# mitsuba-renderer/mitsuba

Measured on AMD Instinct MI355X. Metric: Msamples/s, higher is better.
Workload: dtype f32; 1 GPU; cornell_1024x1024_256spp; scene=cornell_box, triangles=32, width=1024, height=1024, spp=256, integrator=path_hip maxDepth=-1 rrDepth=5, rfilter=gaussian stddev 0.5, sampler=ctr seed 0, block_size=32, parallelism=1 GPU

## Files before the change

### mitsuba_amd/csrc/k_mega.h

```cpp

#ifndef MEGA_PROFILE
#define MEGA_PROFILE 0
#endif
#ifndef MEGA_MB_DIAG
#define MEGA_MB_DIAG 0
#endif
#ifndef MEGA_MB_CLASSES
#define MEGA_MB_CLASSES 1
#endif
#ifndef MEGA_MB_THRESH
#define MEGA_MB_THRESH 40
#endif
#ifndef MEGA_MB_PATIENCE
#define MEGA_MB_PATIENCE 6
#endif
#define MB_NR 48u
template <bool RBOX, uint32_t N> struct MailboxEntry {
    enum { SEQ_ROW = 64 };
    enum { HEAD = 0, DIR = 4, THR = RBOX ? 8 : 7, MIS = THR + 4, ID = MIS + 2, PIXEL, K, STATE, ACCUM, LAST = ACCUM + 3, SEQ = 22 };
    static_assert(LAST < SEQ && SEQ + 2 == MB_DW && MB_DW == 24, "a mailbox entry: the path's state lies below the two rows of the sequence index, which end the MB_DW rows k_pool.h sizes the boxes with");
    static __device__ __forceinline__ void put(uint32_t *x, int row, float f) { x[row * N] = pm_to_bits(f); }
    static __device__ __forceinline__ float get(const uint32_t *x, int row) { return pm_from_bits(x[row * N]); }
    static __device__ __forceinline__ void put4(uint32_t *x, int row, const float4 &f) { put(x, row, f.x); put(x, row + 1, f.y); put(x, row + 2, f.z); put(x, row + 3, f.w); }
    static __device__ __forceinline__ float4 get4(const uint32_t *x, int row) { return make_float4(get(x, row), get(x, row + 1), get(x, row + 2), get(x, row + 3)); }
    template <bool QMC> static __device__ __forceinline__ void store(uint32_t *x, const PathVertex &v, const float4 &accum, const uint32_t *seq) {
        if (RBOX) { put4(x, HEAD, v.rayO); put4(x, DIR, v.rayD); }
        else { put4(x, HEAD, v.hit); put(x, DIR, v.rayD.x); put(x, DIR + 1, v.rayD.y); put(x, DIR + 2, v.rayD.z); }
        put4(x, THR, v.thr);
        put(x, MIS, v.mis.x); put(x, MIS + 1, v.mis.y);
        x[ID * N] = v.id; x[PIXEL * N] = v.pixel; x[K * N] = v.k; x[STATE * N] = v.state;
        put4(x, ACCUM, accum);
        if (QMC) { x[SEQ * N] = seq[0]; x[(SEQ + 1) * N] = seq[SEQ_ROW]; }
    }
    template <bool QMC> static __device__ __forceinline__ void load(const uint32_t *x, PathVertex &v, float4 &accum, uint32_t *seq) {
        if (RBOX) { v.rayO = get4(x, HEAD); v.rayD = get4(x, DIR); }
        else { v.hit = get4(x, HEAD); v.rayD = make_float4(get(x, DIR), get(x, DIR + 1), get(x, DIR + 2), 0.0f); }
        v.thr = get4(x, THR);
        v.mis = make_float2(get(x, MIS), get(x, MIS + 1));
        v.id = x[ID * N]; v.pixel = x[PIXEL * N]; v.k = x[K * N]; v.state = x[STATE * N];
        accum = get4(x, ACCUM);
        if (QMC) { seq[0] = x[SEQ * N]; seq[SEQ_ROW] = x[(SEQ + 1) * N]; }
    }
};
typedef MailboxEntry<false, MB_NS> SBoxEntry;
typedef MailboxEntry<true, MB_NR> RBoxEntry;
static_assert((BLOCK / 64u) * BAL_WAVE_BYTES + MB_DW * MB_NS * sizeof(uint32_t) <= MEGA_DEAL_DWORDS * BLOCK * sizeof(uint32_t), "the S-box lies behind the work lists in the region phip.hip sizes with MEGA_DEAL_DWORDS");
#define MEGA_CHUNK_MAX 4096u
#define MEGA_CHUNK_MIN 64u

enum { MC_SAMPLES = 0, MC_VERTICES, MC_RAYS, MC_NODE, MC_TRI, MC_SH_RAYS, MC_SH_NODE, MC_SH_TRI, MC_COUNT };

template <int MM, bool STRICT, int FLAT ,
          bool QMC ,
          bool DIRECT = false > __global__ __launch_bounds__(BLOCK, MEGA_WAVES) void k_mega(DevScene S, MegaParams M, RenderConst rc, float4 *L) {
    constexpr bool WIDE = FLAT >= 4;
    constexpr bool MAILBOX = MM != 0 && !WIDE && !DIRECT;
    __shared__ uint32_t mbR[MAILBOX ? MB_DW * MB_NR : 1u];
    __shared__ uint32_t mbState[MAILBOX ? MB_NS + MB_NR : 1u];
    __shared__ int mbLive;
    constexpr bool WCNT = (WIDE || (MAILBOX && QMC)) && !MEGA_PROFILE && !MEGA_MB_DIAG;
    __shared__ uint32_t ldsCount[WCNT ? 1 : MC_COUNT][WCNT ? 1 : BLOCK];
#define MEGA_COUNT(row, amount) ldsCount[row][threadIdx.x] += (uint32_t) (amount)
    enum { WC_SAMPLES = 0, WC_VERTICES, WC_RAYS, WC_STEPS, WC_SH_RAYS, WC_SH_STEPS, WC_COUNT };
    __shared__ unsigned long long wcnt[WCNT || WIDE ? BLOCK / 64 : 1][WC_COUNT];
    constexpr int RQ_ROWS = QMC ? 10 : 8;
    __shared__ uint32_t ldsRegen[BLOCK / 64][RQ_ROWS][64];
    __shared__ uint32_t ldsSeq[QMC ? BLOCK / 64 : 1][2][64];
    constexpr uint32_t WAVE_BYTES = WP_WAVE_BYTES;
    unsigned char *wideDeal = g_smem + widePoolDealOffset(M.nodeCache);
    float4 *ldsTriShade = (float4 *) (g_smem + recordsLdsEndOf(S));
    float *ldsEm = WIDE ? (float *) (wideDeal + (BLOCK / 64u) * WAVE_BYTES + (MAILBOX ? MB_DW * MB_NS * sizeof(uint32_t) : 0u))
                        : (float *) (ldsTriShade + (size_t) S.nTriangles * TRISHADE_FLOAT4S);
    DevMaterial *ldsMat = (DevMaterial *) (ldsEm + ((S.emitterTabSize + 3u) & ~3u));
    ShadeTables tab = stageShadeTables<FLAT != 5>(S, ldsEm, ldsMat);
    tab.T.t = ldsEm; tab.materials = FLAT == 5 ? S.materials : ldsMat;
    float4 *ldsFlat = (float4 *) (((uintptr_t) (ldsMat + S.nMaterials) + 15u) & ~(uintptr_t) 15u);
    if (!WIDE) for (uint32_t i = threadIdx.x; i < 2u * S.nFlatLeaves; i += BLOCK) ldsFlat[i] = S.flatLeaves[i];
    lds_cf4 *flat = (lds_cf4 *) ldsFlat; (void) flat;
    if (!WIDE) {
        for (uint32_t i = threadIdx.x; i < S.nTriangles * TRISHADE_FLOAT4S; i += BLOCK) ldsTriShade[i] = S.triShade[i];
        S.triShade = ldsTriShade;
    }
    if (MAILBOX) { if (threadIdx.x < MB_NS + MB_NR) mbState[threadIdx.x] = 0u; if (threadIdx.x == 0u) mbLive = 0; }
    lds_cf4 *const ldsTris = (lds_cf4 *) (g_smem + (size_t) S.dealDwords * BLOCK * sizeof(uint32_t)); (void) ldsTris;
    WidePool wpool;
    if (WIDE) setupWidePool(S, M.nodeCache, g_smem, M.spill + (size_t) blockIdx.x * BLOCK * SPILL_DEPTH, (uint32_t) __builtin_amdgcn_readfirstlane((int) (threadIdx.x >> 6)), wpool);
    else stageRecords(S, g_smem);

    const uint32_t waveId = blockIdx.x * (BLOCK / 64) + (uint32_t) __builtin_amdgcn_readfirstlane((int) (threadIdx.x >> 6)), lane = __lane_id();
    unsigned long long next = 0, end = 0;
    const uint32_t waveInBlock = (uint32_t) __builtin_amdgcn_readfirstlane((int) (threadIdx.x >> 6));
    unsigned char *const waveDeal = wideDeal + waveInBlock * WAVE_BYTES;
    WaveBalance wb = waveBalanceAt(g_smem, waveInBlock);
    if (WIDE) { wb.slot = (lds_u64 *) waveDeal; wb.list = (lds_u16 *) (waveDeal + 2u * 64u * 8u); }
    bool poolOverflow = false;
    uint32_t qHead = 0, qCount = 0;
    V3 camO;
    { V3 d_; float mn_, mx_; cameraRay(S.cam, 0.5f, 0.5f, camO, d_, mn_, mx_); }
    bool exhausted = rc.totalIds == 0;
    uint32_t *mbS = WIDE ? (uint32_t *) (wideDeal + (BLOCK / 64u) * WAVE_BYTES)
                         : (uint32_t *) (g_smem + (BLOCK / 64u) * BAL_WAVE_BYTES);
    const bool server = MAILBOX && waveInBlock == 0u;
    bool haveHit = false;
    uint32_t idleSpins = 0, patience = 0, idleSig = 0;
    bool mbTimedOut = false;
#if MEGA_MB_DIAG
    uint32_t dgDeposit = 0, dgLocal = 0, dgWithdrawn = 0, dgKept = 0, dgServerPass = 0, dgClientPass = 0, dgRefill = 0, dgServerRegen = 0;
#endif
    auto mbAssign = [&](bool wants, bool avail, uint32_t &e) -> bool {
        const unsigned long long am = __ballot(avail), wm = __ballot(wants);
        lds_u32 *map = (lds_u32 *) wb.slot;
        if (avail) map[__builtin_amdgcn_mbcnt_hi((uint32_t) (am >> 32), __builtin_amdgcn_mbcnt_lo((uint32_t) am, 0u))] = lane;
        BAL_SYNC();
        const uint32_t rw = __builtin_amdgcn_mbcnt_hi((uint32_t) (wm >> 32), __builtin_amdgcn_mbcnt_lo((uint32_t) wm, 0u));
        const bool got = wants && rw < (uint32_t) __popcll(am);
        e = got ? map[rw] : 0u;
        BAL_SYNC();
        return got;
    };

    bool alive = false;
    PathVertex v; v.id = v.pixel = v.k = v.state = 0;
    v.hit = v.rayO = v.rayD = v.thr = make_float4(0, 0, 0, 0); v.mis = make_float2(0, 0);
    float4 accum = make_float4(0, 0, 0, 0);
    float4 camHit = make_float4(0, 0, 0, 0);
    if (!WCNT) {
#pragma unroll
        for (int i = 0; i < MC_COUNT; ++i) ldsCount[WCNT ? 0 : i][WCNT ? 0 : threadIdx.x] = 0;
    }
    unsigned long long *const wc = wcnt[(WCNT || WIDE) ? waveInBlock : 0u];
    if ((WCNT || WIDE) && lane < (uint32_t) WC_COUNT) wc[lane] = 0ull;
    auto wcAdd = [&](int row, uint32_t perLane, bool shiftHigh) {
        uint32_t t = perLane;
        t += (uint32_t) __builtin_amdgcn_update_dpp(0, (int) t, 0x111, 0xf, 0xf, true);
        t += (uint32_t) __builtin_amdgcn_update_dpp(0, (int) t, 0x112, 0xf, 0xf, true);
        t += (uint32_t) __builtin_amdgcn_update_dpp(0, (int) t, 0x114, 0xf, 0xf, true);
        t += (uint32_t) __builtin_amdgcn_update_dpp(0, (int) t, 0x118, 0xf, 0xf, true);
        t += (uint32_t) __builtin_amdgcn_update_dpp(0, (int) t, 0x142, 0xa, 0xf, false);
        t += (uint32_t) __builtin_amdgcn_update_dpp(0, (int) t, 0x143, 0xc, 0xf, false);
        if (lane == 63u) wc[row] += shiftHigh ? ((unsigned long long) t << 32) : (unsigned long long) t;
    };
    bool cPush = false, cPend = false;
    float4 cPark = make_float4(0, 0, 0, 0);
    ShadowEntry cSh; cSh.e0 = cSh.e1 = cSh.e2 = make_float4(0, 0, 0, 0);

#if MEGA_PROFILE
    unsigned long long pfT[4] = { 0, 0, 0, 0 }, pfL[4] = { 0, 0, 0, 0 }, pfIter = 0;
// ... 64 lines not shown
                        const bool stop = __hip_atomic_load(M.cancel, __ATOMIC_RELAXED, __HIP_MEMORY_SCOPE_SYSTEM) != 0;
                        if (seen < rc.totalIds && !stop) {
                            const unsigned long long share = (rc.totalIds - seen) / (2ull * M.nWaves);
                            chunk = (uint32_t) (share > MEGA_CHUNK_MAX ? MEGA_CHUNK_MAX : (share < MEGA_CHUNK_MIN ? MEGA_CHUNK_MIN : share));
                            chunk &= ~63u;
                            if (MAILBOX) {
                                atomicAdd(&mbLive, (int) chunk);
                                __builtin_amdgcn_fence(__ATOMIC_SEQ_CST, "workgroup");
                            }
                            base = atomicAdd(M.nextId, (unsigned long long) chunk);
                        } else {
                            base = rc.totalIds;
                        }
                    }
                    const uint32_t blo = __builtin_amdgcn_readfirstlane((uint32_t) base), bhi = __builtin_amdgcn_readfirstlane((uint32_t) (base >> 32));
                    chunk = __builtin_amdgcn_readfirstlane(chunk);
                    next = ((unsigned long long) bhi << 32) | blo;
                    end = next + chunk; if (end > rc.totalIds) end = rc.totalIds;
                    if (MAILBOX && lane == 0u && chunk) {
                        const unsigned long long granted = end > next ? end - next : 0ull;
                        if (granted < chunk) atomicSub(&mbLive, (int) (chunk - granted));
                    }
                    if (next >= end) { exhausted = true; break; }
                }
                const unsigned long long id = next + lane;
                uint32_t px = 0, py = 0, k = 0;
                const bool valid = id < end && decodeId(rc, S.film, id, px, py, k);
                const unsigned long long vmask = __ballot(valid);
                if (MAILBOX) { const int skipped = __popcll(__ballot(id < end && !valid)); if (skipped && lane == 0u) atomicSub(&mbLive, skipped); }
                if (valid) {
                    const uint32_t pos = __builtin_amdgcn_mbcnt_hi((uint32_t) (vmask >> 32), __builtin_amdgcn_mbcnt_lo((uint32_t) vmask, 0u));
                    const uint32_t pixel = py * (uint32_t) S.film.width + px;
                    const V2 jit = streamJitter<QMC>(rc, pixel, k, (uint32_t) S.film.width);
                    if (QMC && rc.jitter) rc.jitter[id] = make_float2(jit.x, jit.y);
                    const float sx = (float) px + jit.x, sy = (float) py + jit.y;
                    V3 o, d; float mint, maxt;
                    cameraRay(S.cam, sx, sy, o, d, mint, maxt);
                    uint32_t *q = &ldsRegen[waveInBlock][0][pos];
                    q[0 * 64] = pm_to_bits(mint);
                    q[1 * 64] = pm_to_bits(d.x); q[2 * 64] = pm_to_bits(d.y); q[3 * 64] = pm_to_bits(d.z); q[4 * 64] = pm_to_bits(maxt);
                    q[5 * 64] = (uint32_t) id; q[6 * 64] = pixel; q[7 * 64] = k;
                    if (QMC) {
                        const uint64_t sidx = isSequenceSampler(rc.sampler) ? seqIndex(rc, k, px, py) : 0ull;
                        q[8 * 64] = (uint32_t) sidx; q[9 * 64] = (uint32_t) (sidx >> 32);
                    }
                }
                qHead = 0u; qCount = (uint32_t) __popcll(vmask);
                next = (end - next < 64ull) ? end : next + 64ull;
                if (qCount == 0u) continue;
            }
            const uint32_t rank = __builtin_amdgcn_mbcnt_hi((uint32_t) (want >> 32), __builtin_amdgcn_mbcnt_lo((uint32_t) want, 0u));
            if (!alive && rank < qCount) {
                const uint32_t *q = &ldsRegen[waveInBlock][0][qHead + rank];
                v.rayO = make_float4(camO.x, camO.y, camO.z, pm_from_bits(q[0 * 64]));
                v.rayD = make_float4(pm_from_bits(q[1 * 64]), pm_from_bits(q[2 * 64]), pm_from_bits(q[3 * 64]), pm_from_bits(q[4 * 64]));
                v.id = q[5 * 64]; v.pixel = q[6 * 64]; v.k = q[7 * 64];
                if (QMC) { ldsSeq[waveInBlock][0][lane] = q[8 * 64]; ldsSeq[waveInBlock][1][lane] = q[9 * 64]; }
                v.thr = make_float4(1.0f, 1.0f, 1.0f, 1.0f);
                v.mis = make_float2(0.0f, 0.0f);
                v.state = 1u | F_ALIVE | F_EMITTED | F_FIRST;
                accum = make_float4(0, 0, 0, 0);
                alive = true;
            }
            const uint32_t wanted = (uint32_t) __popcll(want), took = wanted < qCount ? wanted : qCount;
            qHead += took; qCount -= took;
        }
        PF_END(0, pfWant_) }
        if (MAILBOX) {
            if (!__any(alive)) {
                const int live_ = __hip_atomic_load(&mbLive, __ATOMIC_ACQUIRE, __HIP_MEMORY_SCOPE_WORKGROUP);
                if (exhausted && qCount == 0u && live_ <= 0) break;
                {
                    const uint32_t stS_ = __hip_atomic_load(&mbState[lane], __ATOMIC_RELAXED, __HIP_MEMORY_SCOPE_WORKGROUP);
                    const uint32_t stR_ = lane < MB_NR ? __hip_atomic_load(&mbState[MB_NS + lane], __ATOMIC_RELAXED, __HIP_MEMORY_SCOPE_WORKGROUP) : 0u;
                    const unsigned long long fs_ = __ballot(stS_ == 2u), fr_ = __ballot(stR_ == 2u);
                    const uint32_t sig_ = (uint32_t) live_ * 0x9E3779B9u ^ (uint32_t) fs_ ^ (uint32_t) (fs_ >> 32) * 3u ^ (uint32_t) fr_ * 5u ^ (uint32_t) (fr_ >> 32) * 7u;
                    if (sig_ != idleSig) { idleSig = sig_; idleSpins = 0u; }
                }
                if (++idleSpins > (1u << 22)) { mbTimedOut = true; break; }
                __builtin_amdgcn_s_sleep(8);
                continue;
            }
            idleSpins = 0;
        } else if (!__any(alive || (WIDE && cPush))) break;

        uint32_t hitCls = 0;
        { PF_BEGIN
        const V3 o(v.rayO.x, v.rayO.y, v.rayO.z), d(v.rayD.x, v.rayD.y, v.rayD.z);
        float mint, maxt;
        TravResult r;
        V3 rcp;
        const bool trace = alive && !(MAILBOX && haveHit) && !(DIRECT && (v.state & F_NOTRACE));
        const bool go = trace & clipToSceneSel<false>(S, o, d, v.rayO.w, v.rayD.w, mint, maxt, rcp);
        if (WIDE) {
            const V3 so(cSh.e0.x, cSh.e0.y, cSh.e0.z), sd(cSh.e1.x, cSh.e1.y, cSh.e1.z);
            float smint = 0.0f, smaxt = 0.0f;
            V3 srcp; const bool goS = cPush & clipToSceneSel<true>(S, so, sd, PT_EPSILON, cSh.e0.w, smint, smaxt, srcp);
            bool occluded = false;
            traceWidePool<true, true>(S, wpool, lane, goS, so, sd, smint, smaxt, go, o, d, mint, maxt, occluded, r, wc + WC_SH_STEPS, wc + WC_STEPS, poolOverflow);
            if (trace) {
                v.hit = make_float4(r.t, r.u, r.v, pm_from_bits(r.prim));
                hitCls = r.cls;
            }
            { const uint32_t n_ = (uint32_t) __popcll(__ballot(trace)); if (lane == 0u) wc[WC_RAYS] += n_; }
            if (cPush && !occluded) {
                if (cPend) { cPark.x += cSh.e2.x; cPark.y += cSh.e2.y; cPark.z += cSh.e2.z; }
                else { accum.x += cSh.e2.x; accum.y += cSh.e2.y; accum.z += cSh.e2.z; }
            }
            if (cPend) L[pm_to_bits(cSh.e2.w)] = cPark;
            const uint32_t nS_ = (uint32_t) __popcll(__ballot(cPush)), nE_ = (uint32_t) __popcll(__ballot(cPend));
            if (lane == 0u) { wc[WC_SH_RAYS] += nS_; wc[WC_SAMPLES] += nE_; }
            cPush = false; cPend = false;
        } else {
            uint32_t nNode = 0, nTri = 0;
            traverseFlat2W<false, FLAT == 3>(flat, S.nFlatLeaves, ldsTris, wb, lane, go, o, d, rcp, mint, maxt, r, nNode, nTri);
            if (trace) {
                v.hit = make_float4(r.t, r.u, r.v, pm_from_bits(r.prim));
                hitCls = r.cls;
                if (!WCNT) { MEGA_COUNT(MC_RAYS, 1); MEGA_COUNT(MC_NODE, nNode); MEGA_COUNT(MC_TRI, nTri); }
            }
            if (WCNT) { wcAdd(WC_RAYS, trace ? 1u : 0u, false); wcAdd(WC_STEPS, trace ? nNode : 0u, false); wcAdd(WC_STEPS, trace ? nTri : 0u, true); }
        }

        PF_END(1, __ballot(alive)) }
        if (MAILBOX && !server) {
            const bool special = alive && pm_to_bits(v.hit.w) != PHIP_NO_HIT && hitCls != 0u && ((MEGA_MB_CLASSES >> (hitCls - 1u)) & 1u);
            if (__any(special)) {
                const uint32_t stt = __hip_atomic_load(&mbState[lane], __ATOMIC_ACQUIRE, __HIP_MEMORY_SCOPE_WORKGROUP);
                uint32_t e;
                const bool got = mbAssign(special, stt == 0u && (lane * 3u) / MB_NS == waveInBlock - 1u, e);
                if (got) {
                    SBoxEntry::store<QMC>(mbS + e, v, accum, &ldsSeq[QMC ? waveInBlock : 0][0][lane]);
                    __hip_atomic_store(&mbState[e], 2u, __ATOMIC_RELEASE, __HIP_MEMORY_SCOPE_WORKGROUP);
                    alive = false;
#if MEGA_MB_DIAG
                    ++dgDeposit;
#endif
                }
#if MEGA_MB_DIAG
                if (special && alive) ++dgLocal;
#endif
            }
#if MEGA_MB_DIAG
            if (lane == 0u) ++dgClientPass;
#endif
        }
#if MEGA_MB_DIAG
        if (MAILBOX && server && lane == 0u) ++dgServerPass;
        if (MAILBOX && server && alive && !haveHit && (v.state & F_FIRST)) ++dgServerRegen;
#endif
        bool pushShadow = false, ended = false;
        ShadowEntry sh;
        sh.e0 = sh.e1 = make_float4(0, 0, 0, 0);
        { PF_BEGIN
        if (alive) {
            uint32_t nv = 0;
            bool newRay;
            const LRegister acc{ accum, (QMC && isSequenceSampler(rc.sampler)) ? &ldsSeq[QMC ? waveInBlock : 0][0][lane] : nullptr };
            if (DIRECT) ended = directVertex<MM, QMC ? 8 : 0>(S, tab.T, tab.materials, rc, v, camHit, acc, newRay, pushShadow, sh, nv);
            else ended = shadeVertex<MM, STRICT, QMC ? 8 : 0>(S, tab.T, tab.materials, rc, v, acc, newRay, pushShadow, sh, nv);
            if (ended) { if (WCNT) atomicAdd(&wc[WC_VERTICES], (unsigned long long) nv); else MEGA_COUNT(MC_VERTICES, nv); }
        }

        PF_END(2, __ballot(alive)) }
        { PF_BEGIN
        if (WIDE) {
            cPush = pushShadow; cSh = sh;
            if (ended) {
                if (pushShadow) { cPark = accum; cPend = true; }
                else L[v.id] = accum;
                alive = false;
            }
            const uint32_t n_ = (uint32_t) __popcll(__ballot(ended && !pushShadow));
            if (lane == 0u) wc[WC_SAMPLES] += n_;
        } else {
            const V3 o(sh.e0.x, sh.e0.y, sh.e0.z), d(sh.e1.x, sh.e1.y, sh.e1.z);
            float mint, maxt;
            TravResult r;
            uint32_t nNode = 0, nTri = 0;
            V3 rcp;
            const bool go = pushShadow & clipToSceneSel<true>(S, o, d, PT_EPSILON, sh.e0.w, mint, maxt, rcp);
            const bool occluded = traverseFlat2W<true, FLAT == 3>(flat, S.nFlatLeaves, ldsTris, wb, lane, go, o, d, rcp, mint, maxt, r, nNode, nTri);
            if (pushShadow) {
                if (!WCNT) { MEGA_COUNT(MC_SH_RAYS, 1); MEGA_COUNT(MC_SH_NODE, nNode); MEGA_COUNT(MC_SH_TRI, nTri); }
                if (!occluded) { accum.x += sh.e2.x; accum.y += sh.e2.y; accum.z += sh.e2.z; }
            }
            if (WCNT) { wcAdd(WC_SH_RAYS, pushShadow ? 1u : 0u, false); wcAdd(WC_SH_STEPS, pushShadow ? nNode : 0u, false); wcAdd(WC_SH_STEPS, pushShadow ? nTri : 0u, true); }
        }

        PF_END(3, __ballot(pushShadow)) }
        if (ended && !WIDE) {
            L[v.id] = accum;
            if (!WCNT) MEGA_COUNT(MC_SAMPLES, 1);
            alive = false;
        }
        if (WCNT && !WIDE) { const uint32_t n_ = (uint32_t) __popcll(__ballot(ended)); if (lane == 0u) wc[WC_SAMPLES] += n_; }
        if (MAILBOX) {
            const int nEnded = __popcll(__ballot(ended));
            if (nEnded && lane == 0u) atomicSub(&mbLive, nEnded);
            if (server && __any(alive)) {
                const uint32_t stt = lane < MB_NR ? __hip_atomic_load(&mbState[MB_NS + lane], __ATOMIC_ACQUIRE, __HIP_MEMORY_SCOPE_WORKGROUP) : ~0u;
                uint32_t e;
                if (mbAssign(alive, stt == 0u, e)) {
                    RBoxEntry::store<QMC>(mbR + e, v, accum, &ldsSeq[QMC ? waveInBlock : 0][0][lane]);
                    __hip_atomic_store(&mbState[MB_NS + e], 2u, __ATOMIC_RELEASE, __HIP_MEMORY_SCOPE_WORKGROUP);
                    alive = false;
                }
#if MEGA_MB_DIAG
                if (alive) ++dgKept;
#endif
            }
        }
    }
#if MEGA_PROFILE
    if (lane == 0) {
        ldsCount[MC_RAYS][threadIdx.x] = (uint32_t) (pfT[0] >> 8); ldsCount[MC_NODE][threadIdx.x] = (uint32_t) (pfT[1] >> 8); ldsCount[MC_TRI][threadIdx.x] = (uint32_t) (pfT[2] >> 8);
        ldsCount[MC_SH_RAYS][threadIdx.x] = (uint32_t) (pfT[3] >> 8);
        ldsCount[MC_SH_NODE][threadIdx.x] = (uint32_t) pfL[1]; ldsCount[MC_SH_TRI][threadIdx.x] = (uint32_t) pfL[2]; ldsCount[MC_VERTICES][threadIdx.x] = (uint32_t) pfL[3];
        ldsCount[MC_SAMPLES][threadIdx.x] = (uint32_t) pfIter;
    } else {
#pragma unroll
        for (int i = 0; i < MC_COUNT; ++i) ldsCount[i][threadIdx.x] = 0;
    }
#endif

#if MEGA_MB_DIAG
    ldsCount[MC_NODE][threadIdx.x] = dgDeposit; ldsCount[MC_TRI][threadIdx.x] = dgLocal; ldsCount[MC_SH_NODE][threadIdx.x] = dgWithdrawn; ldsCount[MC_SH_TRI][threadIdx.x] = dgKept;
    ldsCount[MC_RAYS][threadIdx.x] = dgServerPass; ldsCount[MC_SH_RAYS][threadIdx.x] = dgClientPass; ldsCount[MC_VERTICES][threadIdx.x] = dgRefill; ldsCount[MC_SAMPLES][threadIdx.x] = dgServerRegen;
#endif
    PathPool P; P.stat = M.stat; P.nWaves = M.nWaves;
    bool gaveUp = __any((MAILBOX && mbTimedOut) || (WIDE && poolOverflow));
#if MEGA_MB_FAULT
    const bool faulty = M.faultWaves == 3u || (M.faultWaves == 2u && waveId < BLOCK / 64u) || (M.faultWaves == 1u && waveId == 0u);
    if (faulty && M.faultShort != 2u) gaveUp = true;
#endif
    const int rows[MC_COUNT] = { ST_SAMPLES, ST_VERTICES, ST_CLOSEST_RAYS, ST_NODE, ST_TRI, ST_SHADOW_RAYS, ST_SH_NODE, ST_SH_TRI };
#pragma unroll
    for (int i = 0; i < MC_COUNT; ++i) {
        unsigned long long val = 0ull;
        if (WCNT) {
            if (lane == 0u)
                val = i == MC_SAMPLES ? wc[WC_SAMPLES] : i == MC_VERTICES ? wc[WC_VERTICES] : i == MC_RAYS ? wc[WC_RAYS] : i == MC_NODE ? (wc[WC_STEPS] & 0xFFFFFFFFull)
                    : i == MC_TRI ? (wc[WC_STEPS] >> 32) : i == MC_SH_RAYS ? wc[WC_SH_RAYS] : i == MC_SH_NODE ? (wc[WC_SH_STEPS] & 0xFFFFFFFFull) : (wc[WC_SH_STEPS] >> 32);
        } else val = ldsCount[WCNT ? 0 : i][WCNT ? 0 : threadIdx.x];
#if MEGA_MB_FAULT
        if (i == MC_SAMPLES && faulty && M.faultShort && lane == 0u) val -= 1ull;
#endif
        waveStat(P, rows[i], waveId, val);
    }
    if (gaveUp && lane == 0u) P.stat[(size_t) ST_GAVE_UP * P.nWaves + waveId] = 1ull;
}
```

### mitsuba_amd/csrc/k_traverse.h

```cpp

struct TravResult { float t, u, v; uint32_t prim; uint32_t cls = 0;  };

typedef __attribute__((address_space(3))) uint32_t lds_u32;
typedef float f4v __attribute__((ext_vector_type(4)));
typedef const __attribute__((address_space(3))) f4v lds_cf4;
__device__ __forceinline__ float4 ldsLoad4(lds_cf4 *p) { const f4v v = *p; return make_float4(v.x, v.y, v.z, v.w); }

#define MEGA_DEAL_DWORDS 12u
__host__ __device__ __forceinline__ size_t recordsLdsEndOf(const DevScene &S) {
    return (size_t) S.dealDwords * BLOCK * sizeof(uint32_t) + (size_t) S.triCache * 3 * sizeof(float4);
}
__host__ __device__ __forceinline__ size_t megaLdsBytesOf(const DevScene &S) {
    return recordsLdsEndOf(S) + (size_t) S.nTriangles * TRISHADE_FLOAT4S * sizeof(float4) + (size_t) ((S.emitterTabSize + 3u) & ~3u) * sizeof(float)
         + (size_t) S.nMaterials * sizeof(DevMaterial) + 16  + (size_t) S.nFlatLeaves * 2 * sizeof(float4);
}

__host__ __device__ __forceinline__ size_t shadeTraceLdsBytes(const DevScene &S) {
    return (size_t) S.nFlatLeaves * 2 * sizeof(float4) + (size_t) S.triCache * 3 * sizeof(float4) + (size_t) ((S.emitterTabSize + 3u) & ~3u) * sizeof(float)
         + (size_t) S.nMaterials * sizeof(DevMaterial);
}

__device__ __forceinline__ lds_cf4 *stageRecords(const DevScene &S, unsigned char *smem) {
    float4 *lt = (float4 *) (smem + (size_t) S.dealDwords * BLOCK * sizeof(uint32_t));
    for (uint32_t i = threadIdx.x; i < S.triCache * 3u; i += BLOCK)
        lt[i] = S.tris[i];
    __syncthreads();
    return (lds_cf4 *) lt;
}

#define SPILL_DEPTH 96


typedef float f2v __attribute__((ext_vector_type(2)));
__device__ __forceinline__ bool waldIntersectSel(const float4 &a, const float4 &b, const float4 &c, const V3 &o, const V3 &d,
                                                 float mint, float maxt, float &u, float &v, float &t) {
    const uint32_t k = pm_to_bits(a.x);
    const bool k0 = k == 0, k2 = k == 2;
    const float o_u = k0 ? o.y : (k2 ? o.x : o.z), o_v = k0 ? o.z : (k2 ? o.y : o.x), o_k = k0 ? o.x : (k2 ? o.z : o.y);
    const float d_u = k0 ? d.y : (k2 ? d.x : d.z), d_v = k0 ? d.z : (k2 ? d.y : d.x), d_k = k0 ? d.x : (k2 ? d.z : d.y);
    const float n_u = a.y, n_v = a.z, n_d = a.w;
    t = (n_d - o_u * n_u - o_v * n_v - o_k) / (d_u * n_u + d_v * n_v + d_k);
    const float hu = o_u + t * d_u - b.x;
    const float hv = o_v + t * d_v - b.y;
    u = hv * b.z + hu * b.w;
    v = hu * c.x + hv * c.y;
    return (k < 3u) & !(t < mint) & !(t > maxt) & (u >= 0) & (v >= 0) & (u + v <= 1.0f);
}


template <bool R64 = false>
__device__ __forceinline__ uint32_t flat2Pass1(lds_cf4 *flat, uint32_t nFlat, const V3 &o, const V3 &rcp, float mint, float maxt, uint32_t *maskHi = nullptr) {
    uint32_t mask = 0, hi = 0;
    const f2v rxy = { rcp.x, rcp.y }, oxy = { -(o.x * rcp.x), -(o.y * rcp.y) };
    const f2v rz2 = { rcp.z, 0.0f }, oz2 = { -(o.z * rcp.z), 0.0f };
    f2v axy = { fabsf(rcp.x), fabsf(rcp.y) }, az2 = { fabsf(rcp.z), 0.0f };
    asm("" : "+v"(axy), "+v"(az2));
#define FLAT2_BOX(c_)                                                                                                                  \
        {                                                                                                                              \
            const f4v A = flat[2 * (c_)], B = flat[2 * (c_) + 1];                                                                      \
            const f2v cxy = __builtin_elementwise_fma(A.xy, rxy, oxy), cz = __builtin_elementwise_fma(A.zw, rz2, oz2);                 \
            f2v tx, ty, tz;                                                                 \
            asm("v_pk_fma_f32 %0, %1, %2, %3 op_sel_hi:[0,0,0] neg_lo:[1,0,0]" : "=v"(tx) : "v"(B.xy), "v"(axy), "v"(cxy));            \
            asm("v_pk_fma_f32 %0, %1, %2, %3 op_sel:[1,1,1] op_sel_hi:[1,1,1] neg_lo:[1,0,0]" : "=v"(ty) : "v"(B.xy), "v"(axy), "v"(cxy)); \
            asm("v_pk_fma_f32 %0, %1, %2, %3 op_sel_hi:[0,0,0] neg_lo:[1,0,0]" : "=v"(tz) : "v"(B.zw), "v"(az2), "v"(cz));             \
            float tn, tf;                                                                                                              \
            asm("v_max3_f32 %0, %1, %2, %3" : "=v"(tn) : "v"(tx.x), "v"(ty.x), "v"(mint));                                              \
            asm("v_max_f32 %0, %1, %2" : "=v"(tn) : "v"(tn), "v"(tz.x));                                                               \
            asm("v_min3_f32 %0, %1, %2, %3" : "=v"(tf) : "v"(tx.y), "v"(ty.y), "v"(maxt));                                              \
            asm("v_min_f32 %0, %1, %2" : "=v"(tf) : "v"(tf), "v"(tz.y));                                                               \
            mask |= (tn <= tf) ? pm_to_bits(B.w) : 0u;                                                                                 \
            if (R64) hi |= (tn <= tf) ? pm_to_bits(A.w) : 0u;                                                                          \
        }
    const uint32_t nFlat4 = nFlat & ~3u;
    for (uint32_t c4 = 0; c4 < nFlat4; c4 += 4) {
#pragma unroll
        for (uint32_t j = 0; j < 4; ++j) FLAT2_BOX(c4 + j)
    }
    for (uint32_t c = nFlat4; c < nFlat; ++c) FLAT2_BOX(c)
#undef FLAT2_BOX
    if (R64) *maskHi = hi;
    return mask;
}


#define BAL_CAP 512u
#ifndef BAL_ILP
#define BAL_ILP 1
#endif
#define BAL_WAVE_BYTES (64u * 8u + BAL_CAP * 2u)
typedef __attribute__((address_space(3))) uint16_t lds_u16;
typedef __attribute__((address_space(3))) unsigned long long lds_u64;
struct WaveBalance { lds_u64 *slot; lds_u16 *list; };
__device__ __forceinline__ WaveBalance waveBalanceAt(unsigned char *smem, uint32_t waveInBlock) {
    unsigned char *p = smem + waveInBlock * BAL_WAVE_BYTES;
    WaveBalance wb; wb.slot = (lds_u64 *) p; wb.list = (lds_u16 *) (p + 64u * 8u);
    return wb;
}
#define BAL_SYNC() { __builtin_amdgcn_fence(__ATOMIC_SEQ_CST, "wavefront"); __builtin_amdgcn_wave_barrier(); }

template <bool R64> struct RecMask;
template <> struct RecMask<false> { typedef uint32_t T; static __device__ __forceinline__ uint32_t popc(T m) { return (uint32_t) __popc(m); }
                                    static __device__ __forceinline__ uint32_t ctz(T m) { return (uint32_t) __builtin_ctz(m); }
                                    static __device__ __forceinline__ T upTo(uint32_t i) { return (2u << i) - 1u; } };
template <> struct RecMask<true>  { typedef unsigned long long T; static __device__ __forceinline__ uint32_t popc(T m) { return (uint32_t) __popcll(m); }
                                    static __device__ __forceinline__ uint32_t ctz(T m) { return (uint32_t) __builtin_ctzll(m); }
                                    static __device__ __forceinline__ T upTo(uint32_t i) { return i >= 63u ? ~0ull : (2ull << i) - 1ull; } };
template <bool SHADOW, bool R64 = false>
__device__ __forceinline__ bool traverseFlat2W(lds_cf4 *flat, uint32_t nFlat, lds_cf4 *tris, const WaveBalance &wb, uint32_t lane, bool go,
                                               const V3 &o, const V3 &d, const V3 &rcp, float mint, float maxt, TravResult &res, uint32_t &nodeVisits, uint32_t &triTests) {
    typedef RecMask<R64> RM; typedef typename RM::T Mask;
    constexpr uint32_t RB = R64 ? 6u : 5u, RMSK = (1u << RB) - 1u;
    uint32_t maskHi = 0;
    const uint32_t maskLo = flat2Pass1<R64>(flat, nFlat, o, rcp, mint, maxt, &maskHi);
    Mask mask = R64 ? (Mask) (((unsigned long long) maskHi << 32) | maskLo) : (Mask) maskLo;
    mask = go ? mask : (Mask) 0;
    nodeVisits += go ? 1u : 0u;
    const Mask mask0 = mask;

    if (SHADOW) *(lds_u32 *) (wb.slot + lane) = 0xFFFFFFFFu; else wb.slot[lane] = ~0ull;
    while (__ballot(mask != 0)) {
        const uint32_t pc = RM::popc(mask);
        uint32_t incl = pc;
        incl += (uint32_t) __builtin_amdgcn_update_dpp(0, (int) incl, 0x111 , 0xf, 0xf, true);
        incl += (uint32_t) __builtin_amdgcn_update_dpp(0, (int) incl, 0x112 , 0xf, 0xf, true);
        incl += (uint32_t) __builtin_amdgcn_update_dpp(0, (int) incl, 0x114 , 0xf, 0xf, true);
        incl += (uint32_t) __builtin_amdgcn_update_dpp(0, (int) incl, 0x118 , 0xf, 0xf, true);
        incl += (uint32_t) __builtin_amdgcn_update_dpp(0, (int) incl, 0x142 , 0xa, 0xf, false);
        incl += (uint32_t) __builtin_amdgcn_update_dpp(0, (int) incl, 0x143 , 0xc, 0xf, false);
        const bool fits = incl <= BAL_CAP;
        const uint32_t nFit = (uint32_t) __popcll(__ballot(fits));
        const uint32_t total = (uint32_t) __builtin_amdgcn_readlane((int) incl, (int) (nFit - 1u));
        if (pc && fits) {
            const uint32_t tag = lane << RB;
            lds_u16 *w = wb.list + (incl - pc);
            do {
                *w++ = (uint16_t) (tag | RM::ctz(mask));
                mask &= mask - 1u;
            } while (mask);
        }
        BAL_SYNC()
        for (uint32_t base = 0; base < total; base += 64u * BAL_ILP) {
            bool hit[BAL_ILP]; uint32_t own[BAL_ILP], lo[BAL_ILP], hi[BAL_ILP];
#pragma unroll
            for (uint32_t j = 0; j < BAL_ILP; ++j) {
                const uint32_t i = base + 64u * j + lane;
                const uint32_t item = wb.list[i];
                const uint32_t owner = (item >> RB) & 63u, rec = item & RMSK;
                const int src = (int) (owner << 2);
                const V3 po(pm_from_bits((uint32_t) __builtin_amdgcn_ds_bpermute(src, (int) pm_to_bits(o.x))), pm_from_bits((uint32_t) __builtin_amdgcn_ds_bpermute(src, (int) pm_to_bits(o.y))),
                            pm_from_bits((uint32_t) __builtin_amdgcn_ds_bpermute(src, (int) pm_to_bits(o.z))));
                const V3 pd(pm_from_bits((uint32_t) __builtin_amdgcn_ds_bpermute(src, (int) pm_to_bits(d.x))), pm_from_bits((uint32_t) __builtin_amdgcn_ds_bpermute(src, (int) pm_to_bits(d.y))),
                            pm_from_bits((uint32_t) __builtin_amdgcn_ds_bpermute(src, (int) pm_to_bits(d.z))));
                const float pmint = pm_from_bits((uint32_t) __builtin_amdgcn_ds_bpermute(src, (int) pm_to_bits(mint)));
                const float pmaxt = pm_from_bits((uint32_t) __builtin_amdgcn_ds_bpermute(src, (int) pm_to_bits(maxt)));
                lds_cf4 *t_ = tris + 3 * rec;
                const float4 a = ldsLoad4(t_), b = ldsLoad4(t_ + 1), c = ldsLoad4(t_ + 2);
                float tu, tv, tt;
                hit[j] = (i < total) & waldIntersectSel(a, b, c, po, pd, pmint, pmaxt, tu, tv, tt);
                own[j] = owner; hi[j] = pm_to_bits(tt);
                lo[j] = SHADOW ? rec : ((((0xFFFFFFFFu >> RB) - pm_to_bits(c.z)) << RB) | rec);
            }
#pragma unroll
            for (uint32_t j = 0; j < BAL_ILP; ++j)
                if (hit[j]) {
                    if (SHADOW) __hip_atomic_fetch_min((lds_u32 *) (wb.slot + own[j]), lo[j], __ATOMIC_RELAXED, __HIP_MEMORY_SCOPE_WORKGROUP);
                    else __hip_atomic_fetch_min(wb.slot + own[j], ((unsigned long long) hi[j] << 32) | (unsigned long long) lo[j], __ATOMIC_RELAXED, __HIP_MEMORY_SCOPE_WORKGROUP);
                }
        }
        BAL_SYNC()
    }
    res.prim = PHIP_NO_HIT; res.t = INFINITY; res.u = res.v = 0;
    if (SHADOW) {
        const uint32_t first = *(lds_u32 *) (wb.slot + lane);
        const bool found = first != 0xFFFFFFFFu;
        triTests += RM::popc(found ? (Mask) (mask0 & RM::upTo(first & RMSK)) : mask0);
        return found;
    } else {
        const unsigned long long best = wb.slot[lane];
        const bool found = best != ~0ull;
        triTests += RM::popc(mask0);
        lds_cf4 *t_ = tris + 3 * ((uint32_t) best & RMSK);
        const float4 a = ldsLoad4(t_), b = ldsLoad4(t_ + 1), c = ldsLoad4(t_ + 2);
        const float tt = pm_from_bits((uint32_t) (best >> 32));
        const uint32_t k = pm_to_bits(a.x);
        const bool k0 = k == 0, k2 = k == 2;
        const float o_u = k0 ? o.y : (k2 ? o.x : o.z), o_v = k0 ? o.z : (k2 ? o.y : o.x);
        const float d_u = k0 ? d.y : (k2 ? d.x : d.z), d_v = k0 ? d.z : (k2 ? d.y : d.x);
        const float hu = o_u + tt * d_u - b.x, hv = o_v + tt * d_v - b.y;
        const float tu = hv * b.z + hu * b.w, tv = hu * c.x + hv * c.y;
        res.t = found ? tt : res.t; res.u = found ? tu : res.u; res.v = found ? tv : res.v; res.prim = found ? pm_to_bits(c.z) : res.prim;
        res.cls = found ? (pm_to_bits(c.w) & 3u) : 0u;
        return found;
    }
}

extern __shared__ __attribute__((aligned(16))) unsigned char g_smem[];
```

Measured before the change: 4605 Msamples/s.

## Defer shadow rays and trace them jointly with next bounce in flat traversal

Extends the deferred-shadow scheme, used before only by the wide path, to the flat non-mailbox non-QMC path. Each iteration now traces the pending shadow ray and the closest-hit ray together. A shared box pass and a joint work-balanced triangle list replace two separate traversals, so the wave runs one balancing loop instead of two. The cost is extra LDS per wave for a separate shadow slot, a larger deal size, and more bpermutes per item.

```diff
diff --git a/mitsuba_amd/csrc/k_joint_list.h b/mitsuba_amd/csrc/k_joint_list.h
--- /dev/null
+++ b/mitsuba_amd/csrc/k_joint_list.h
@@ -0,0 +1,13 @@
+#pragma once
+#include <stdint.h>
+#if defined(__HIPCC__) || defined(__CUDACC__)
+#define JL_FN __host__ __device__ __forceinline__
+#else
+#define JL_FN static inline
+#endif
+JL_FN uint32_t jointCounts(uint32_t pairsS, uint32_t pairsC) { return pairsS | (pairsC << 16); }
+JL_FN uint32_t jointCountS(uint32_t packed) { return packed & 0xFFFFu; }
+JL_FN uint32_t jointCountC(uint32_t packed) { return packed >> 16; }
+JL_FN bool jointFits(uint32_t inclPacked, uint32_t cap) { return jointCountS(inclPacked) + jointCountC(inclPacked) <= cap; }
+JL_FN uint32_t jointOffsetS(uint32_t inclPacked, uint32_t pairsS) { return jointCountS(inclPacked) - pairsS; }
+JL_FN uint32_t jointOffsetC(uint32_t inclPacked, uint32_t pairsC, uint32_t totalS) { return totalS + jointCountC(inclPacked) - pairsC; }
diff --git a/mitsuba_amd/csrc/k_mega.h b/mitsuba_amd/csrc/k_mega.h
--- a/mitsuba_amd/csrc/k_mega.h
+++ b/mitsuba_amd/csrc/k_mega.h
@@ -63,6 +63,7 @@
 #define MEGA_COUNT(row, amount) ldsCount[row][threadIdx.x] += (uint32_t) (amount)
     enum { WC_SAMPLES = 0, WC_VERTICES, WC_RAYS, WC_STEPS, WC_SH_RAYS, WC_SH_STEPS, WC_COUNT };
     __shared__ unsigned long long wcnt[WCNT || WIDE ? BLOCK / 64 : 1][WC_COUNT];
+    constexpr bool DEFER = WIDE || (!MAILBOX && !DIRECT && !QMC);
     constexpr int RQ_ROWS = QMC ? 10 : 8;
     __shared__ uint32_t ldsRegen[BLOCK / 64][RQ_ROWS][64];
     __shared__ uint32_t ldsSeq[QMC ? BLOCK / 64 : 1][2][64];
@@ -293,7 +294,7 @@
                 continue;
             }
             idleSpins = 0;
-        } else if (!__any(alive || (WIDE && cPush))) break;
+        } else if (!__any(alive || (DEFER && cPush))) break;
 
         uint32_t hitCls = 0;
         { PF_BEGIN
@@ -303,24 +304,31 @@
         V3 rcp;
         const bool trace = alive && !(MAILBOX && haveHit) && !(DIRECT && (v.state & F_NOTRACE));
         const bool go = trace & clipToSceneSel<false>(S, o, d, v.rayO.w, v.rayD.w, mint, maxt, rcp);
-        if (WIDE) {
+        if (DEFER) {
             const V3 so(cSh.e0.x, cSh.e0.y, cSh.e0.z), sd(cSh.e1.x, cSh.e1.y, cSh.e1.z);
             float smint = 0.0f, smaxt = 0.0f;
             V3 srcp; const bool goS = cPush & clipToSceneSel<true>(S, so, sd, PT_EPSILON, cSh.e0.w, smint, smaxt, srcp);
             bool occluded = false;
-            traceWidePool<true, true>(S, wpool, lane, goS, so, sd, smint, smaxt, go, o, d, mint, maxt, occluded, r, wc + WC_SH_STEPS, wc + WC_STEPS, poolOverflow);
+            uint32_t nNode = 0, nTri = 0, sNode = 0, sTri = 0;
+            if (WIDE) traceWidePool<true, true>(S, wpool, lane, goS, so, sd, smint, smaxt, go, o, d, mint, maxt, occluded, r, wc + WC_SH_STEPS, wc + WC_STEPS, poolOverflow);
+            else traverseFlat2J<FLAT == 3>(flat, S.nFlatLeaves, ldsTris, wb, lane, goS, so, sd, srcp, smint, smaxt, go, o, d, rcp, mint, maxt, occluded, r, sNode, sTri, nNode, nTri);
             if (trace) {
                 v.hit = make_float4(r.t, r.u, r.v, pm_from_bits(r.prim));
                 hitCls = r.cls;
             }
-            { const uint32_t n_ = (uint32_t) __popcll(__ballot(trace)); if (lane == 0u) wc[WC_RAYS] += n_; }
             if (cPush && !occluded) {
                 if (cPend) { cPark.x += cSh.e2.x; cPark.y += cSh.e2.y; cPark.z += cSh.e2.z; }
                 else { accum.x += cSh.e2.x; accum.y += cSh.e2.y; accum.z += cSh.e2.z; }
             }
             if (cPend) L[pm_to_bits(cSh.e2.w)] = cPark;
-            const uint32_t nS_ = (uint32_t) __popcll(__ballot(cPush)), nE_ = (uint32_t) __popcll(__ballot(cPend));
-            if (lane == 0u) { wc[WC_SH_RAYS] += nS_; wc[WC_SAMPLES] += nE_; }
+            if (WIDE) {
+                const uint32_t n_ = (uint32_t) __popcll(__ballot(trace)), nS_ = (uint32_t) __popcll(__ballot(cPush)), nE_ = (uint32_t) __popcll(__ballot(cPend));
+                if (lane == 0u) { wc[WC_RAYS] += n_; wc[WC_SH_RAYS] += nS_; wc[WC_SAMPLES] += nE_; }
+            } else {
+                if (trace) { MEGA_COUNT(MC_RAYS, 1); MEGA_COUNT(MC_NODE, nNode); MEGA_COUNT(MC_TRI, nTri); }
+                if (cPush) { MEGA_COUNT(MC_SH_RAYS, 1); MEGA_COUNT(MC_SH_NODE, sNode); MEGA_COUNT(MC_SH_TRI, sTri); }
+                if (cPend) MEGA_COUNT(MC_SAMPLES, 1);
+            }
             cPush = false; cPend = false;
         } else {
             uint32_t nNode = 0, nTri = 0;
@@ -375,15 +383,15 @@
 
         PF_END(2, __ballot(alive)) }
         { PF_BEGIN
-        if (WIDE) {
+        if (DEFER) {
             cPush = pushShadow; cSh = sh;
             if (ended) {
                 if (pushShadow) { cPark = accum; cPend = true; }
                 else L[v.id] = accum;
                 alive = false;
             }
-            const uint32_t n_ = (uint32_t) __popcll(__ballot(ended && !pushShadow));
-            if (lane == 0u) wc[WC_SAMPLES] += n_;
+            if (WIDE) { const uint32_t n_ = (uint32_t) __popcll(__ballot(ended && !pushShadow)); if (lane == 0u) wc[WC_SAMPLES] += n_; }
+            else if (ended && !pushShadow) MEGA_COUNT(MC_SAMPLES, 1);
         } else {
             const V3 o(sh.e0.x, sh.e0.y, sh.e0.z), d(sh.e1.x, sh.e1.y, sh.e1.z);
             float mint, maxt;
@@ -400,12 +408,12 @@
         }
 
         PF_END(3, __ballot(pushShadow)) }
-        if (ended && !WIDE) {
+        if (ended && !DEFER) {
             L[v.id] = accum;
             if (!WCNT) MEGA_COUNT(MC_SAMPLES, 1);
             alive = false;
         }
-        if (WCNT && !WIDE) { const uint32_t n_ = (uint32_t) __popcll(__ballot(ended)); if (lane == 0u) wc[WC_SAMPLES] += n_; }
+        if (WCNT && !DEFER) { const uint32_t n_ = (uint32_t) __popcll(__ballot(ended)); if (lane == 0u) wc[WC_SAMPLES] += n_; }
         if (MAILBOX) {
             const int nEnded = __popcll(__ballot(ended));
             if (nEnded && lane == 0u) atomicSub(&mbLive, nEnded);
diff --git a/mitsuba_amd/csrc/k_traverse.h b/mitsuba_amd/csrc/k_traverse.h
--- a/mitsuba_amd/csrc/k_traverse.h
+++ b/mitsuba_amd/csrc/k_traverse.h
@@ -6,7 +6,7 @@
 typedef const __attribute__((address_space(3))) f4v lds_cf4;
 __device__ __forceinline__ float4 ldsLoad4(lds_cf4 *p) { const f4v v = *p; return make_float4(v.x, v.y, v.z, v.w); }
 
-#define MEGA_DEAL_DWORDS 12u
+#define MEGA_DEAL_DWORDS 13u
 __host__ __device__ __forceinline__ size_t recordsLdsEndOf(const DevScene &S) {
     return (size_t) S.dealDwords * BLOCK * sizeof(uint32_t) + (size_t) S.triCache * 3 * sizeof(float4);
 }
@@ -48,28 +48,40 @@
 }
 
 
-template <bool R64 = false>
-__device__ __forceinline__ uint32_t flat2Pass1(lds_cf4 *flat, uint32_t nFlat, const V3 &o, const V3 &rcp, float mint, float maxt, uint32_t *maskHi = nullptr) {
-    uint32_t mask = 0, hi = 0;
-    const f2v rxy = { rcp.x, rcp.y }, oxy = { -(o.x * rcp.x), -(o.y * rcp.y) };
-    const f2v rz2 = { rcp.z, 0.0f }, oz2 = { -(o.z * rcp.z), 0.0f };
-    f2v axy = { fabsf(rcp.x), fabsf(rcp.y) }, az2 = { fabsf(rcp.z), 0.0f };
-    asm("" : "+v"(axy), "+v"(az2));
+struct Flat2Ray { f2v rxy, oxy, rz2, oz2, axy, az2; };
+__device__ __forceinline__ Flat2Ray flat2Ray(const V3 &o, const V3 &rcp) {
+    Flat2Ray q;
+    q.rxy = f2v{ rcp.x, rcp.y }; q.oxy = f2v{ -(o.x * rcp.x), -(o.y * rcp.y) };
+    q.rz2 = f2v{ rcp.z, 0.0f }; q.oz2 = f2v{ -(o.z * rcp.z), 0.0f };
+    q.axy = f2v{ fabsf(rcp.x), fabsf(rcp.y) }; q.az2 = f2v{ fabsf(rcp.z), 0.0f };
+    asm("" : "+v"(q.axy), "+v"(q.az2));
+    return q;
+}
+__device__ __forceinline__ bool flat2Enters(const f4v &A, const f4v &B, const Flat2Ray &q, float mint, float maxt) {
+    const f2v cxy = __builtin_elementwise_fma(A.xy, q.rxy, q.oxy), cz = __builtin_elementwise_fma(A.zw, q.rz2, q.oz2);
+    f2v tx, ty, tz;
+    asm("v_pk_fma_f32 %0, %1, %2, %3 op_sel_hi:[0,0,0] neg_lo:[1,0,0]" : "=v"(tx) : "v"(B.xy), "v"(q.axy), "v"(cxy));
+    asm("v_pk_fma_f32 %0, %1, %2, %3 op_sel:[1,1,1] op_sel_hi:[1,1,1] neg_lo:[1,0,0]" : "=v"(ty) : "v"(B.xy), "v"(q.axy), "v"(cxy));
+    asm("v_pk_fma_f32 %0, %1, %2, %3 op_sel_hi:[0,0,0] neg_lo:[1,0,0]" : "=v"(tz) : "v"(B.zw), "v"(q.az2), "v"(cz));
+    float tn, tf;
+    asm("v_max3_f32 %0, %1, %2, %3" : "=v"(tn) : "v"(tx.x), "v"(ty.x), "v"(mint));
+    asm("v_max_f32 %0, %1, %2" : "=v"(tn) : "v"(tn), "v"(tz.x));
+    asm("v_min3_f32 %0, %1, %2, %3" : "=v"(tf) : "v"(tx.y), "v"(ty.y), "v"(maxt));
+    asm("v_min_f32 %0, %1, %2" : "=v"(tf) : "v"(tf), "v"(tz.y));
+    return tn <= tf;
+}
+template <bool R64, int N>
+__device__ __forceinline__ void flat2Pass1N(lds_cf4 *flat, uint32_t nFlat, const Flat2Ray (&q)[N], const float (&mint)[N], const float (&maxt)[N], uint32_t (&mask)[N], uint32_t (&hi)[N]) {
+#pragma unroll
+    for (int n = 0; n < N; ++n) mask[n] = hi[n] = 0u;
 #define FLAT2_BOX(c_)                                                                                                                  \
         {                                                                                                                              \
             const f4v A = flat[2 * (c_)], B = flat[2 * (c_) + 1];                                                                      \
-            const f2v cxy = __builtin_elementwise_fma(A.xy, rxy, oxy), cz = __builtin_elementwise_fma(A.zw, rz2, oz2);                 \
-            f2v tx, ty, tz;                                                                 \
-            asm("v_pk_fma_f32 %0, %1, %2, %3 op_sel_hi:[0,0,0] neg_lo:[1,0,0]" : "=v"(tx) : "v"(B.xy), "v"(axy), "v"(cxy));            \
-            asm("v_pk_fma_f32 %0, %1, %2, %3 op_sel:[1,1,1] op_sel_hi:[1,1,1] neg_lo:[1,0,0]" : "=v"(ty) : "v"(B.xy), "v"(axy), "v"(cxy)); \
-            asm("v_pk_fma_f32 %0, %1, %2, %3 op_sel_hi:[0,0,0] neg_lo:[1,0,0]" : "=v"(tz) : "v"(B.zw), "v"(az2), "v"(cz));             \
-            float tn, tf;                                                                                                              \
-            asm("v_max3_f32 %0, %1, %2, %3" : "=v"(tn) : "v"(tx.x), "v"(ty.x), "v"(mint));                                              \
-            asm("v_max_f32 %0, %1, %2" : "=v"(tn) : "v"(tn), "v"(tz.x));                                                               \
-            asm("v_min3_f32 %0, %1, %2, %3" : "=v"(tf) : "v"(tx.y), "v"(ty.y), "v"(maxt));                                              \
-            asm("v_min_f32 %0, %1, %2" : "=v"(tf) : "v"(tf), "v"(tz.y));                                                               \
-            mask |= (tn <= tf) ? pm_to_bits(B.w) : 0u;                                                                                 \
-            if (R64) hi |= (tn <= tf) ? pm_to_bits(A.w) : 0u;                                                                          \
+            _Pragma("unroll") for (int n = 0; n < N; ++n) {                                                                            \
+                const bool in = flat2Enters(A, B, q[n], mint[n], maxt[n]);                                                             \
+                mask[n] |= in ? pm_to_bits(B.w) : 0u;                                                                                  \
+                if (R64) hi[n] |= in ? pm_to_bits(A.w) : 0u;                                                                           \
+            }                                                                                                                          \
         }
     const uint32_t nFlat4 = nFlat & ~3u;
     for (uint32_t c4 = 0; c4 < nFlat4; c4 += 4) {
@@ -78,22 +90,30 @@
     }
     for (uint32_t c = nFlat4; c < nFlat; ++c) FLAT2_BOX(c)
 #undef FLAT2_BOX
-    if (R64) *maskHi = hi;
-    return mask;
+}
+template <bool R64 = false>
+__device__ __forceinline__ uint32_t flat2Pass1(lds_cf4 *flat, uint32_t nFlat, const V3 &o, const V3 &rcp, float mint, float maxt, uint32_t *maskHi = nullptr) {
+    const Flat2Ray q[1] = { flat2Ray(o, rcp) };
+    const float mn[1] = { mint }, mx[1] = { maxt };
+    uint32_t mask[1], hi[1];
+    flat2Pass1N<R64, 1>(flat, nFlat, q, mn, mx, mask, hi);
+    if (R64) *maskHi = hi[0];
+    return mask[0];
 }
 
 
 #define BAL_CAP 512u
+#include "k_joint_list.h"
 #ifndef BAL_ILP
 #define BAL_ILP 1
 #endif
-#define BAL_WAVE_BYTES (64u * 8u + BAL_CAP * 2u)
+#define BAL_WAVE_BYTES (64u * 8u + BAL_CAP * 2u + 64u * 4u)
 typedef __attribute__((address_space(3))) uint16_t lds_u16;
 typedef __attribute__((address_space(3))) unsigned long long lds_u64;
-struct WaveBalance { lds_u64 *slot; lds_u16 *list; };
+struct WaveBalance { lds_u64 *slot; lds_u16 *list; lds_u32 *slotS; };
 __device__ __forceinline__ WaveBalance waveBalanceAt(unsigned char *smem, uint32_t waveInBlock) {
     unsigned char *p = smem + waveInBlock * BAL_WAVE_BYTES;
-    WaveBalance wb; wb.slot = (lds_u64 *) p; wb.list = (lds_u16 *) (p + 64u * 8u);
+    WaveBalance wb; wb.slot = (lds_u64 *) p; wb.list = (lds_u16 *) (p + 64u * 8u); wb.slotS = (lds_u32 *) (p + 64u * 8u + BAL_CAP * 2u);
     return wb;
 }
 #define BAL_SYNC() { __builtin_amdgcn_fence(__ATOMIC_SEQ_CST, "wavefront"); __builtin_amdgcn_wave_barrier(); }
@@ -105,6 +125,30 @@
 template <> struct RecMask<true>  { typedef unsigned long long T; static __device__ __forceinline__ uint32_t popc(T m) { return (uint32_t) __popcll(m); }
                                     static __device__ __forceinline__ uint32_t ctz(T m) { return (uint32_t) __builtin_ctzll(m); }
                                     static __device__ __forceinline__ T upTo(uint32_t i) { return i >= 63u ? ~0ull : (2ull << i) - 1ull; } };
+template <bool R64> __device__ __forceinline__ bool flat2AnyHit(uint32_t first, typename RecMask<R64>::T mask0, uint32_t &triTests) {
+    typedef RecMask<R64> RM; typedef typename RM::T Mask;
+    const bool found = first != 0xFFFFFFFFu;
+    triTests += RM::popc(found ? (Mask) (mask0 & RM::upTo(first & ((R64 ? 64u : 32u) - 1u))) : mask0);
+    return found;
+}
+template <bool R64> __device__ __forceinline__ bool flat2Closest(unsigned long long best, typename RecMask<R64>::T mask0, lds_cf4 *tris, const V3 &o, const V3 &d, TravResult &res, uint32_t &triTests) {
+    typedef RecMask<R64> RM;
+    res.prim = PHIP_NO_HIT; res.t = INFINITY; res.u = res.v = 0;
+    const bool found = best != ~0ull;
+    triTests += RM::popc(mask0);
+    lds_cf4 *t_ = tris + 3 * ((uint32_t) best & ((R64 ? 64u : 32u) - 1u));
+    const float4 a = ldsLoad4(t_), b = ldsLoad4(t_ + 1), c = ldsLoad4(t_ + 2);
+    const float tt = pm_from_bits((uint32_t) (best >> 32));
+    const uint32_t k = pm_to_bits(a.x);
+    const bool k0 = k == 0, k2 = k == 2;
+    const float o_u = k0 ? o.y : (k2 ? o.x : o.z), o_v = k0 ? o.z : (k2 ? o.y : o.x);
+    const float d_u = k0 ? d.y : (k2 ? d.x : d.z), d_v = k0 ? d.z : (k2 ? d.y : d.x);
+    const float hu = o_u + tt * d_u - b.x, hv = o_v + tt * d_v - b.y;
+    const float tu = hv * b.z + hu * b.w, tv = hu * c.x + hv * c.y;
+    res.t = found ? tt : res.t; res.u = found ? tu : res.u; res.v = found ? tv : res.v; res.prim = found ? pm_to_bits(c.z) : res.prim;
+    res.cls = found ? (pm_to_bits(c.w) & 3u) : 0u;
+    return found;
+}
 template <bool SHADOW, bool R64 = false>
 __device__ __forceinline__ bool traverseFlat2W(lds_cf4 *flat, uint32_t nFlat, lds_cf4 *tris, const WaveBalance &wb, uint32_t lane, bool go,
                                                const V3 &o, const V3 &d, const V3 &rcp, float mint, float maxt, TravResult &res, uint32_t &nodeVisits, uint32_t &triTests) {
@@ -169,29 +213,93 @@
         }
         BAL_SYNC()
     }
-    res.prim = PHIP_NO_HIT; res.t = INFINITY; res.u = res.v = 0;
-    if (SHADOW) {
-        const uint32_t first = *(lds_u32 *) (wb.slot + lane);
-        const bool found = first != 0xFFFFFFFFu;
-        triTests += RM::popc(found ? (Mask) (mask0 & RM::upTo(first & RMSK)) : mask0);
-        return found;
-    } else {
-        const unsigned long long best = wb.slot[lane];
-        const bool found = best != ~0ull;
-        triTests += RM::popc(mask0);
-        lds_cf4 *t_ = tris + 3 * ((uint32_t) best & RMSK);
-        const float4 a = ldsLoad4(t_), b = ldsLoad4(t_ + 1), c = ldsLoad4(t_ + 2);
-        const float tt = pm_from_bits((uint32_t) (best >> 32));
-        const uint32_t k = pm_to_bits(a.x);
-        const bool k0 = k == 0, k2 = k == 2;
-        const float o_u = k0 ? o.y : (k2 ? o.x : o.z), o_v = k0 ? o.z : (k2 ? o.y : o.x);
-        const float d_u = k0 ? d.y : (k2 ? d.x : d.z), d_v = k0 ? d.z : (k2 ? d.y : d.x);
-        const float hu = o_u + tt * d_u - b.x, hv = o_v + tt * d_v - b.y;
-        const float tu = hv * b.z + hu * b.w, tv = hu * c.x + hv * c.y;
-        res.t = found ? tt : res.t; res.u = found ? tu : res.u; res.v = found ? tv : res.v; res.prim = found ? pm_to_bits(c.z) : res.prim;
-        res.cls = found ? (pm_to_bits(c.w) & 3u) : 0u;
-        return found;
+    if (SHADOW) return flat2AnyHit<R64>(*(lds_u32 *) (wb.slot + lane), mask0, triTests);
+    return flat2Closest<R64>(wb.slot[lane], mask0, tris, o, d, res, triTests);
+}
+
+template <bool R64>
+__device__ __forceinline__ void traverseFlat2J(lds_cf4 *flat, uint32_t nFlat, lds_cf4 *tris, const WaveBalance &wb, uint32_t lane,
+                                               bool goS, const V3 &so, const V3 &sd, const V3 &srcp, float smint, float smaxt,
+                                               bool go, const V3 &o, const V3 &d, const V3 &rcp, float mint, float maxt,
+                                               bool &occluded, TravResult &res, uint32_t &nodeVisitsS, uint32_t &triTestsS, uint32_t &nodeVisits, uint32_t &triTests) {
+    typedef RecMask<R64> RM; typedef typename RM::T Mask;
+    constexpr uint32_t RB = R64 ? 6u : 5u, RMSK = (1u << RB) - 1u;
+    Mask maskS, maskC;
+    {
+        const Flat2Ray q[2] = { flat2Ray(so, srcp), flat2Ray(o, rcp) };
+        const float mn[2] = { smint, mint }, mx[2] = { smaxt, maxt };
+        uint32_t lo[2], hi[2];
+        flat2Pass1N<R64, 2>(flat, nFlat, q, mn, mx, lo, hi);
+        maskS = R64 ? (Mask) (((unsigned long long) hi[0] << 32) | lo[0]) : (Mask) lo[0];
+        maskC = R64 ? (Mask) (((unsigned long long) hi[1] << 32) | lo[1]) : (Mask) lo[1];
     }
+    maskS = goS ? maskS : (Mask) 0; maskC = go ? maskC : (Mask) 0;
+    nodeVisitsS += goS ? 1u : 0u; nodeVisits += go ? 1u : 0u;
+    const Mask mask0S = maskS, mask0C = maskC;
+
+    wb.slotS[lane] = 0xFFFFFFFFu; wb.slot[lane] = ~0ull;
+    while (__ballot((maskS | maskC) != 0)) {
+        const uint32_t pcS = RM::popc(maskS), pcC = RM::popc(maskC);
+        uint32_t incl = jointCounts(pcS, pcC);
+        incl += (uint32_t) __builtin_amdgcn_update_dpp(0, (int) incl, 0x111 , 0xf, 0xf, true);
+        incl += (uint32_t) __builtin_amdgcn_update_dpp(0, (int) incl, 0x112 , 0xf, 0xf, true);
+        incl += (uint32_t) __builtin_amdgcn_update_dpp(0, (int) incl, 0x114 , 0xf, 0xf, true);
+        incl += (uint32_t) __builtin_amdgcn_update_dpp(0, (int) incl, 0x118 , 0xf, 0xf, true);
+        incl += (uint32_t) __builtin_amdgcn_update_dpp(0, (int) incl, 0x142 , 0xa, 0xf, false);
+        incl += (uint32_t) __builtin_amdgcn_update_dpp(0, (int) incl, 0x143 , 0xc, 0xf, false);
+        const bool fits = jointFits(incl, BAL_CAP);
+        const uint32_t nFit = (uint32_t) __popcll(__ballot(fits));
+        const uint32_t totals = (uint32_t) __builtin_amdgcn_readlane((int) incl, (int) (nFit - 1u));
+        const uint32_t totalS = jointCountS(totals), total = totalS + jointCountC(totals);
+        if (fits) {
+            const uint32_t tag = lane << RB;
+            if (pcS) {
+                lds_u16 *w = wb.list + jointOffsetS(incl, pcS);
+                do { *w++ = (uint16_t) (tag | RM::ctz(maskS)); maskS &= maskS - 1u; } while (maskS);
+            }
+            if (pcC) {
+                lds_u16 *w = wb.list + jointOffsetC(incl, pcC, totalS);
+                do { *w++ = (uint16_t) (tag | RM::ctz(maskC)); maskC &= maskC - 1u; } while (maskC);
+            }
+        }
+        BAL_SYNC()
+        for (uint32_t base = 0; base < total; base += 64u) {
+            const bool stepS = base < totalS, stepC = base + 64u > totalS;
+            const uint32_t i = base + lane;
+            const bool kindC = i >= totalS;
+            const uint32_t item = wb.list[i];
+            const uint32_t owner = (item >> RB) & 63u, rec = item & RMSK;
+            const int src = (int) (owner << 2);
+            const float mine[2][8] = { { so.x, so.y, so.z, sd.x, sd.y, sd.z, smint, smaxt }, { o.x, o.y, o.z, d.x, d.y, d.z, mint, maxt } };
+            float ray[8];
+#pragma unroll
+            for (int k = 0; k < 8; ++k) ray[k] = 0.0f;
+            if (stepC) {
+#pragma unroll
+                for (int k = 0; k < 8; ++k) ray[k] = pm_from_bits((uint32_t) __builtin_amdgcn_ds_bpermute(src, (int) pm_to_bits(mine[1][k])));
+            }
+            if (stepS) {
+#pragma unroll
+                for (int k = 0; k < 8; ++k) {
+                    const float s_ = pm_from_bits((uint32_t) __builtin_amdgcn_ds_bpermute(src, (int) pm_to_bits(mine[0][k])));
+                    ray[k] = kindC ? ray[k] : s_;
+                }
+            }
+            const V3 po(ray[0], ray[1], ray[2]), pd(ray[3], ray[4], ray[5]);
+            lds_cf4 *t_ = tris + 3 * rec;
+            const float4 a = ldsLoad4(t_), b = ldsLoad4(t_ + 1), c = ldsLoad4(t_ + 2);
+            float tu, tv, tt;
+            const bool hit = (i < total) & waldIntersectSel(a, b, c, po, pd, ray[6], ray[7], tu, tv, tt);
+            if (hit) {
+                if (kindC) __hip_atomic_fetch_min(wb.slot + owner, ((unsigned long long) pm_to_bits(tt) << 32) | (unsigned long long) ((((0xFFFFFFFFu >> RB) - pm_to_bits(c.z)) << RB) | rec),
+                                                  __ATOMIC_RELAXED, __HIP_MEMORY_SCOPE_WORKGROUP);
+                else __hip_atomic_fetch_min(wb.slotS + owner, rec, __ATOMIC_RELAXED, __HIP_MEMORY_SCOPE_WORKGROUP);
+            }
+        }
+        BAL_SYNC()
+    }
+    occluded = flat2AnyHit<R64>(wb.slotS[lane], mask0S, triTestsS);
+    flat2Closest<R64>(wb.slot[lane], mask0C, tris, o, d, res, triTests);
 }
 
 extern __shared__ __attribute__((aligned(16))) unsigned char g_smem[];
```

Measured after the change: 4440 Msamples/s. 3.6% lower.
